# YamaneKoyo/mri-to-speech

Hardware: AMD Instinct MI355X
Metric: rtMRI frames/s end-to-end (256x256 frames -> 64-bin mel -> 11413 Hz wav) (higher is better)
Workload: dtype bf16x3; 1 GPU; e2e rtMRI->wav, 64 clips x 30 frames per GPU at 256x256 (configs[3] per-GPU share); clips_per_gpu=64, frames_per_clip=30, global_batch_clips=64, hw=256, parallelism=dp1, chunk=1920

## Files before the change

mri-to-speech_amd/csrc/acoustic_cnn.cpp:

```cpp
#include <algorithm>

#include "plan_util.hpp"
#include "prof.hpp"

namespace m2s {

Acoustic::Acoustic(const StateDict& sd, int n_mels, int hidden, int dtype, int device)
    : dtype_(dtype), device_(device), n_mels_(n_mels), hidden_(hidden), sw_(Switches::from_env()) {
  pack_acoustic(sd, n_mels, hidden, dtype, arena_, p_);
  arena_.upload(device);
  for (auto& b : p_.blocks) {
    b.c1.resolve(arena_);
    if (b.type != 0) b.c2.resolve(arena_);
    if (b.type == 2) {
      b.se1.resolve(arena_);
      b.se2.resolve(arena_);
    }
  }
  p_.lstm_ih.resolve(arena_);
  M2S_HIP(hipHostMalloc(reinterpret_cast<void**>(&err_host_), sizeof(unsigned), hipHostMallocMapped | hipHostMallocCoherent));
  *err_host_ = 0;
  M2S_HIP(hipHostGetDevicePointer(reinterpret_cast<void**>(&err_dev_), err_host_, 0));
  M2S_HIP(hipMalloc(&gsync_, lstm_sync_bytes(true)));
}
// ... 108 lines not shown
  const Block& b = p_.blocks[k];
  const BlockRoute& r = *p.r;
  const int nc = p.nc, oh = r.oh, ow = r.ow, nh = r.nh, nw = r.nw, qt = r.qt, ql = r.ql;
  T *const cur = p.cur, *const nxt = p.nxt;
  hipStream_t s = p.s;
  const int co = chan_stride(b.cout);
  const double px = (double)nc * nh * nw, flops = 2.0 * px * b.mid * (9.0 * b.cin + b.cout);
  if constexpr (kSplit<T>) {
    switch (r.er) {
      case ErRoute::ErSp:
        launch_er_sp(cur, nc, nh, nw, b.c1.cs_in, b.mid, co, arena_.ptr(b.er_sp_w), b.c1.b, b.c2.b, nxt, flops,
                     4.0 * px * (b.c1.cs_in + co), s, sw_.er_mrg);
        return;
      case ErRoute::Ers2Sp:
        launch_ers2_sp(cur, nc, oh, ow, nh, nw, qt, ql, b.c1.cs_in, b.mid, co, arena_.ptr(b.er_wexp), b.c1.b,
                       arena_.ptr(b.er_wpwl), b.c2.b, nxt, flops, 4.0 * ((double)nc * oh * ow * b.c1.cs_in + px * co), s);
        return;
      default:
        break;
    }
  } else if constexpr (std::is_same<T, bf16_t>::value) {
    const uint8_t* const x8 = r.x8_in ? p.cur8 : nullptr;
    uint8_t* const y8 = p.next8 = r.y8_out ? p.other8() : nullptr;
    switch (r.er) {
      case ErRoute::Er8:
        launch_er8_fused(cur, nc, nh, nw, arena_.at<uint8_t>(b.er8_wexp), arena_.at<float>(b.er8_sexp), b.c1.b,
                         arena_.at<uint8_t>(b.er8_wpwl), arena_.at<float>(b.er8_spwl), b.c2.b, nxt, flops,
                         2.0 * px * (2.0 * b.cin) + (3.0 * 8 * 2048 + 2 * 2048), s, x8, y8);
        return;
      case ErRoute::Er:
        launch_er_fused(cur, nc, nh, nw, arena_.at<bf16_t>(b.er_wexp), b.c1.b, arena_.at<bf16_t>(b.er_wpwl), b.c2.b, nxt,
                        flops, 2.0 * px * (2.0 * b.cin) + 2.0 * (9.0 * 32 * 128 + 128 * 32), s);
        return;
      case ErRoute::Er8w:
        launch_er8w_fused(cur, x8, nc, nh, nw, arena_.at<uint8_t>(b.er8w_w), arena_.at<float>(b.er8w_sexp), b.c1.b,
                          arena_.at<float>(b.er8w_spwl), b.c2.b, nxt, y8, flops,
                          px * (b.cin + 2.0 * b.cin + 2.0 * b.cout + (y8 ? b.cout : 0.0)) + (9.0 * b.cin + b.cout) * b.mid, s);
        return;
      case ErRoute::Er2:
        launch_er2_fused(cur, nc, nh, nw, arena_.at<bf16_t>(b.er_wexp), b.c1.b, b.c2.b, nxt, flops,
                         2.0 * px * (2.0 * b.c1.cs_in) + 2.0 * er2_stage_elems(), s);
        return;
      case ErRoute::Ers2:
        launch_ers2_fused(cur, nc, oh, ow, nh, nw, qt, ql, b.c1.cs_in, b.mid, co, arena_.at<bf16_t>(b.er_wexp), b.c1.b,
                          arena_.at<bf16_t>(b.er_wpwl), b.c2.b, nxt, flops,
                          2.0 * ((double)nc * oh * ow * b.c1.cs_in + px * co) + (y8 ? px * 32 : 0.0), s, y8);
        return;
      default:
        break;
    }
  }
  ConvArgs a = conv2d_args(p, b.c1, cur, p.b.M);
  a.act = ACT_SILU;
  ConvArgs q = pw_args(b.c2, p.b.M, nxt, nc * nh * nw, nh * nw);
  q.res = b.skip ? cur : nullptr;
  if (kSplit<T> && sw_.er_s2_fused && b.stride == 2 && conv_gemm_er_supported(a, q, sw_.conv)) {
    launch_conv_gemm_er(a, q, sw_.conv, s, flops,
                        4.0 * ((double)nc * oh * ow * b.cin + px * b.cout + (9.0 * b.cin + b.cout) * b.mid));
  } else {
    run_conv<T>(a, b.c1, sw_.conv, s);
    run_conv<T>(q, b.c2, sw_.conv, s);
  }
}

template <typename T>
void Acoustic::effnet_ir_front(EffPass<T>& p, size_t k) {
  const Block& b = p_.blocks[k];
  const BlockRoute& r = *p.r;
  const int nc = p.nc, oh = r.oh, ow = r.ow, nh = r.nh, nw = r.nw, qt = r.qt, ql = r.ql;
  T *const cur = p.cur, *const M = p.b.M, *const M2 = p.b.M2, *const se_mean = p.b.se_mean;
  float* const sums = p.b.sums;
  hipStream_t s = p.s;
  const int cs = chan_stride(b.mid);
  constexpr bool SPL = kSplit<T>;
  const bool f8 = r.f8;
  const float *const dw_w = arena_.at<float>(b.dw_w), *const dw_b = arena_.at<float>(b.dw_b);
  const void* wdw = SPL ? dw_w : arena_.ptr(b.dw_w2);
  const double Po = (double)nh * nw, es = SPL ? 4.0 : 2.0;
  auto ir_ws = [&](int ih, int iw, int stride, int OH, int OW, int pad_t, int pad_l) {
    const double Pi = (double)ih * iw;
    launch_ir_ws(cur, nc, ih, iw, b.c1.cs_in, b.c1.kp, cs, b.c1.w, b.c1.b, dw_w, dw_b, M2, se_mean,
                 2.0 * nc * b.mid * (Pi * b.c1.cin + Po * 9),
                 4.0 * nc * Pi * b.c1.cin + 4.0 * b.mid * (b.c1.cin + 11.0) + 4.0 * nc * b.mid, s, ws_report(), stride,
                 OH, OW, pad_t, pad_l, 4.0 * nc * Po * b.mid, r.mid_f32, sw_.irws_parts);
  };
  if (r.convert8) {
    p.cur8 = p.b.X8[0];
    launch_rows_e4m3(cur, (long)nc * oh * ow, b.c1.cs_in, p.cur8, b.f8x_kp, s);
  }
  const uint8_t* const x8 = r.x8_in ? p.cur8 : nullptr;
  const double Pi = (double)oh * ow;
  switch (r.front) {
    case IrFront::IrWs:
      ir_ws(nh, nw, 1, 0, 0, 0, 0);
      break;
    case IrFront::Pwdw:
      launch_ir_pwdw(cur, nc, b.c1.cs_in, b.c1.kp, b.c1.w, b.c1.b, wdw, dw_b, nh, nw, cs, M2, se_mean, SPL,
                     2.0 * nc * Po * b.mid * (b.c1.cin + 9), nc * Po * ((x8 ? 1.0 : es) * b.c1.cin + (f8 ? 1.0 : es) * b.mid),
                     s, f8, x8, x8 ? arena_.ptr(b.f8x_w) : nullptr, x8 ? arena_.at<float>(b.f8x_s) : nullptr, b.f8x_kp);
      break;
    case IrFront::IrWsS2:
      ir_ws(oh, ow, 2, nh, nw, qt, ql);
      break;
    case IrFront::PwdwS2:
      launch_ir_pwdw_s2(cur, nc, b.c1.cs_in, b.c1.kp, b.c1.w, b.c1.b, wdw, dw_b, oh, ow, nh, nw, qt, ql, cs, M2, se_mean,
                        SPL, 2.0 * nc * b.mid * (Pi * b.c1.cin + Po * 9),
                        nc * ((x8 ? 1.0 : es) * Pi * b.c1.cin + (f8 ? 1.0 : es) * Po * b.mid), s, f8, x8,
                        x8 ? arena_.ptr(b.f8x_w) : nullptr, x8 ? arena_.at<float>(b.f8x_s) : nullptr, b.f8x_kp);
      break;
    case IrFront::S2Band: {
      launch_ir_s2band(cur, nc, oh, ow, b.c1.cs_in, b.c1.kp, b.c1.w, b.c1.b, dw_w, dw_b, nh, nw, qt, ql, cs, M2, sums, SPL,
                       2.0 * nc * b.mid * (Pi * 1.125 * b.c1.cin + Po * 9),
                       nc * (es * Pi * b.c1.cs_in + (f8 ? 1.0 : es) * Po * cs), s, f8);
      ProfScope ps(tname<T>("se_mean_kernel"), 0.0, 4.0 * nc * cs * ir_s2band_bands(nh) + es * nc * cs, s);
      launch_se_mean<T>(sums, nc, ir_s2band_bands(nh), cs, 1.0f / (float)(nh * nw), se_mean, s);
      break;
    }
    case IrFront::Unfused: {
      ConvArgs e = pw_args(b.c1, cur, M, nc * oh * ow, oh * ow);
      e.act = ACT_SILU;
      run_conv<T>(e, b.c1, sw_.conv, s);
      {
        ProfScope ps(b.stride == 2 ? tname<T>("dwconv_kernel", ", 2") : tname<T>("dwconv_kernel", ", 1"), 2.0 * nc * nh * nw * b.mid * 9,
                     kStoreBytes<T> * (double)nc * (oh * ow + nh * nw) * b.mid, s);
        launch_dwconv<T>(M, nc, oh, ow, nh, nw, b.stride, qt, ql, b.mid, cs, dw_w, dw_b, M2, sums, s);
      }
      {
        ProfScope ps(tname<T>("se_mean_kernel"), 0.0, 4.0 * nc * cs * dw_pixel_blocks(nh, nw) + kStoreBytes<T> * (double)nc * cs, s);
        launch_se_mean<T>(sums, nc, dw_pixel_blocks(nh, nw), cs, 1.0f / (float)(nh * nw), se_mean, s);
      }
      break;
    }
  }
}

template <typename T>
void Acoustic::effnet_ir_se(EffPass<T>& p, size_t k) {
  const Block& b = p_.blocks[k];
  const int nc = p.nc, cs = chan_stride(b.mid);
  T *const se_mean = p.b.se_mean, *const se_hid = p.b.se_hid, *const scale = p.b.scale;
  hipStream_t s = p.s;
  switch (p.r->se) {
    case IrSe::Excite:
      launch_se_excite(se_mean, nc, b.mid, cs, b.se1.w, b.se1.kp, b.se1.b, b.rd, b.se2.w, b.se2.kp, b.se2.b, scale,
                       kSplit<T>, s);
      break;
    case IrSe::Convs: {
      ConvArgs r1 = pw_args(b.se1, se_mean, se_hid, nc, 1);
      r1.act = ACT_SILU;
      run_conv<T>(r1, b.se1, sw_.conv, s);
      ConvArgs r2 = pw_args(b.se2, se_hid, scale, nc, 1);
      r2.act = ACT_SIGMOID;
      run_conv<T>(r2, b.se2, sw_.conv, s);
      break;
    }
  }
}

template <typename T>
void Acoustic::effnet_ir_pwl(EffPass<T>& p, size_t k) {
  const Block& b = p_.blocks[k];
  const BlockRoute& r = *p.r;
  const int nc = p.nc, nh = r.nh, nw = r.nw, cs = chan_stride(b.mid), co = chan_stride(b.cout);
  T *const cur = p.cur, *const nxt = p.nxt, *const M2 = p.b.M2, *const scale = p.b.scale;
  hipStream_t s = p.s;
  uint8_t* const next8 = p.next8 = r.y8_out ? p.other8() : nullptr;
  const int ld8 = r.ld8;
// ... 133 lines not shown
```

mri-to-speech_amd/csrc/ir_ws.hip:

```cpp
#include <algorithm>
#include <cstdlib>
#include <type_traits>
#include <vector>

#include "kernels.hpp"
#include "lds_dma.hpp"
#include "prof.hpp"

namespace m2s {
namespace {

constexpr int WS_SL = 32;
constexpr int WS_BR = 8;
constexpr int WS_NP = 8;
constexpr int WS_NC = 8;
constexpr int WS_UMAX = 3;

__device__ __forceinline__ int hx_of(int r) { return ((r & 3) << 2) | swz_f((r >> 2) & 3); }

struct WsLayout {
  int XR, TROWS, x_bytes, tile_bytes, w_bytes, total;
};

__host__ __device__ inline int ws_cpp(int cs_in) { return (cs_in * 2 + 255) / 256 * 16; }
__host__ __device__ inline WsLayout ws_layout(int H, int W, int cs_in, int cs_mid, int S = 1) {
  WsLayout L;
  const int cpp = ws_cpp(cs_in), xp = 2 * cpp * 16;
  L.XR = 0;
  for (int r0 = 0; r0 < H; r0 += WS_BR) {
    const int a = r0 > 0 ? r0 - 1 : 0, b = r0 + WS_BR + 1 < H ? r0 + WS_BR + 1 : H;
    L.XR = b - a > L.XR ? b - a : L.XR;
  }
  const int tr = ((H < WS_BR ? H : WS_BR) + 2) * (W + 2);
  L.TROWS = S == 1 ? tr + (20 - tr % 16) % 16 : tr + (21 - tr % 16) % 16;
  L.x_bytes = L.XR * W * xp;
  L.tile_bytes = 2 * 8 * L.TROWS * 16;
  L.w_bytes = 2 * (cs_in / 32) * 4096;
  L.total = L.x_bytes + L.tile_bytes + L.w_bytes + (3 * 320 + 2 * 32) * 4 + cs_mid * 8 + 2 * (cs_mid / WS_SL) * 4 + 128;
  return L;
}

#ifndef IRWS_HAND_END
#define IRWS_HAND_END 2
#endif
#ifndef IRWS_PF_DEEP
#define IRWS_PF_DEEP 1
#endif
#ifndef IRWS_PAIR
#define IRWS_PAIR 1
#endif
#ifndef IRWS_TAPS_AHEAD
#define IRWS_TAPS_AHEAD 1
#endif
#ifndef IRWS_JOINT
#define IRWS_JOINT 1
#endif
#ifndef IRWS_PAR
#define IRWS_PAR 1
#endif
template <int W, int KS, int S>
__global__ void __launch_bounds__(64 * (WS_NP + WS_NC), 1)
    ir_ws_kernel(const bf16_t* __restrict__ x, int N, int H, int cs_mid, const bf16_t* __restrict__ wpw,
                 const float* __restrict__ bpw, const float* __restrict__ wdw, const float* __restrict__ bdw,
                 bf16_t* __restrict__ y, bf16_t* __restrict__ se_mean, unsigned long long* __restrict__ trace,
                 unsigned spin_max, unsigned* __restrict__ err, int pad_t, int pad_l, int fm32, int n_full, int parts) {
  constexpr int par = IRWS_PAR;
  static_assert(S == 1 || (S == 2 && W == 16), "stride 2: the 16-wide maps");
  constexpr int OWS = W / S;
  constexpr int OPB = (WS_BR / S) * OWS;
  constexpr bool HAND_END = IRWS_HAND_END == 2 ? W == 8 : IRWS_HAND_END, TAPS_AHEAD = IRWS_TAPS_AHEAD;
  constexpr bool JOINT = IRWS_JOINT && !HAND_END && (IRWS_JOINT == 2 || S == 2);
  constexpr int CS = KS * 32;
  constexpr int CPP = (CS * 2 + 255) / 256 * 16;
  constexpr int CPR = 2 * CPP;
  constexpr int XP = CPR * 16;
  constexpr int WT = W + 2;
  constexpr int WS_PXL = WS_BR * W / 64;
  extern __shared__ __attribute__((aligned(16))) char smem[];
  const WsLayout Lg = ws_layout(H, W, CS, cs_mid, S);
  const int NB = (H + WS_BR - 1) / WS_BR, NS = cs_mid / WS_SL, P = H * W;
  const int PO = S == 1 ? P : ((H + 1) / 2) * OWS;
  const int PLT = Lg.TROWS * 16;
  char* xs = smem;
  char* tiles = xs + Lg.x_bytes;
  char* wbuf = tiles + Lg.tile_bytes;
  float* wdl = reinterpret_cast<float*>(wbuf + Lg.w_bytes);
  float* bpl = wdl + 3 * 320;
  unsigned long long* sq = reinterpret_cast<unsigned long long*>(bpl + 2 * 32);
  unsigned* sq_n = reinterpret_cast<unsigned*>(sq + cs_mid);
  unsigned* sq_nan = sq_n + cs_mid / WS_SL;
  unsigned* ctr = reinterpret_cast<unsigned*>(smem + Lg.total - 128);
  unsigned* pdone = ctr + 0;
  unsigned* wrdy = ctr + 1;
  unsigned* xrdy = ctr + 2;
  unsigned* tfull = ctr + 3;
  unsigned* poison = ctr + 4;
  unsigned* tfree = ctr + 8;

  const int tid = threadIdx.x, lane = tid & 63;
  const int wave = __builtin_amdgcn_readfirstlane(tid >> 6);
  const int g = lane >> 4, r16 = lane & 15;
  const bool prod = wave < WS_NP;
  const int pw = wave & 1;
  unsigned* const pdone_p = par ? (pw ? ctr + 5 : ctr + 0) : pdone;
  unsigned* const wrdy_p = par ? (pw ? ctr + 6 : ctr + 1) : wrdy;
  const unsigned NPC = par ? WS_NP / 2 : WS_NP;
  const int n_units = n_full + (N - n_full) * parts;
  struct Unit {
    int img, lo, hi;
  };
  auto unit_of = [&](int u) {
    if (u < n_full) return Unit{u, 0, NS};
    const int q = u - n_full, pt = q % parts;
    return Unit{n_full + q / parts, pt * NS / parts, (pt + 1) * NS / parts};
  };
  int T = 0;
  for (int u = blockIdx.x; u < n_units; u += gridDim.x) {
    const Unit un = unit_of(u);
    T += NB * (un.hi - un.lo);
  }

  auto TR = [&](int i, int k) {
#ifdef IRWS_TRACE
    if (trace && blockIdx.x == 0 && i < 64) {
      const unsigned long long t = __builtin_amdgcn_s_memtime();
      if (lane == 0) trace[((i * 2 + (wave >= WS_NP)) * 16 + k) * 64 + (wave & 7)] = t;
    }
#else
    (void)i; (void)k; (void)trace;
#endif
  };
  struct Step {
    int img, band, sl, lo, hi, u;
  };
  auto first_step = [&](int u) {
    const Unit un = unit_of(u);
    return Step{un.img, 0, un.lo, un.lo, un.hi, u};
  };
  auto next_step = [&](Step d) {
    if (++d.sl == d.hi) {
      d.sl = d.lo;
      if (++d.band == NB) d = first_step(d.u + (int)gridDim.x);
    }
    return d;
  };

  if (tid < 32) ctr[tid] = 0u;
  for (int i = tid; i < cs_mid; i += 64 * (WS_NP + WS_NC)) sq[i] = 0ull;
// ... 320 lines not shown
    if (__builtin_amdgcn_readfirstlane(arrived) == (unsigned)(NB * WS_NC - 1) && lane < WS_SL) {
      const unsigned long long t = __hip_atomic_exchange(sq + c0 + sc, 0ull, __ATOMIC_RELAXED, __HIP_MEMORY_SCOPE_WORKGROUP);
      const float m = __fmaf_rn((float)(unsigned)t, 2.3283064365386963e-10f, (float)(int)(t >> 32)) / (float)PO;
      act_st<sp_t>(reinterpret_cast<sp_t*>(se_mean), d.img, cs_mid, c0 + sc, (*poison || sq_nan[d.sl]) ? __builtin_nanf("") : m);
      if (lane == 0) {
        sq_n[d.sl] = 0u;
        sq_nan[d.sl] = 0u;
      }
    }
  };

  __syncthreads();
  if (prod) {
    __builtin_amdgcn_s_setprio(2);
    Step cur = first_step(blockIdx.x);
    if (T > 0) issue_w(0, cur);
    if (T > 1) issue_w(1, next_step(cur));
    if (TAPS_AHEAD && T > 0 && tap_wave) issue_wd(0, cur);
    if (T > 0) {
      wait_vm_le((T > 1 ? npw : 0) + (TAPS_AHEAD && tap_wave ? 1 : 0));
      bump(wrdy_p);
      if (!HAND_END) wait_ge(wrdy_p, NPC);
    }
    static_assert(4 * KS <= 4 * WS_NP, "pieces per wave");
    int bands = 0;
    for (int i = 0; i < T; ++i) {
      const Step nxt = next_step(cur), nxt2 = next_step(nxt);
      TR(i, 0);
      if (cur.sl == cur.lo) {
        if (i > 0) {
          wait_ge(pdone_p, NPC * (unsigned)i);
          if (par) wait_ge(pw ? ctr + 0 : ctr + 5, NPC * (unsigned)i);
        }
        issue_x(cur.img, cur.band);
        wait_vm<0>();
        bump(xrdy);
        wait_ge(xrdy, (unsigned)(WS_NP * ++bands));
      }
      TR(i, 1);
      if (!TAPS_AHEAD && tap_wave) {
        if (i >= 3) wait_all(tfree, (unsigned)(i - 2));
        issue_wd(i, cur);
      }
      if (HAND_END) wait_ge(wrdy_p, NPC * (unsigned)(i + 1));
      TR(i, 2);
      produce(i, cur, nxt2);
      if (HAND_END) {
        wait_vm<0>();
        asm volatile("s_waitcnt lgkmcnt(0)" ::: "memory");
        if (lane == 0) {
          asm volatile("ds_add_u32 %0, %1" ::"v"((uint32_t)(uintptr_t)wrdy_p), "v"(1u) : "memory");
          asm volatile("ds_add_u32 %0, %1" ::"v"((uint32_t)(uintptr_t)tfull), "v"(1u) : "memory");
        }
        TR(i, 12);
        const bool nw = i + 2 < T, nt = TAPS_AHEAD && tap_wave && i + 1 < T;
        if (nw || nt) {
          wait_ge(pdone_p, NPC * (unsigned)(i + 1));
          if (nw) issue_w(i + 2, nxt2);
          if (nt) issue_wd(i + 1, nxt);
        }
      } else {
        if (tap_wave) {
          const bool nt = TAPS_AHEAD && i + 1 < T;
          if (nt) issue_wd(i + 1, nxt);
          wait_vm_le((i + 2 < T ? npw : 0) + (nt ? 1 : 0));
        }
        bump(tfull);
        TR(i, 12);
      }
      TR(i, 3);
      cur = nxt;
    }
  } else {
    Step cur = first_step(blockIdx.x);
    for (int i = 0; i < T; ++i) {
      wait_ge(tfull, (unsigned)(WS_NP * (i + 1)));
      consume(i, cur);
      TR(i, 7);
      cur = next_step(cur);
    }
  }
}

#ifdef IRWS_TRACE
static void dump_trace(unsigned long long* tr, hipStream_t s, const char* tag) {
  static int calls = 0;
  if (++calls > 40) return;
  std::vector<unsigned long long> h(64 * 2 * 16 * 64);
  M2S_HIP(hipStreamSynchronize(s));
  M2S_HIP(hipMemcpy(h.data(), tr, h.size() * 8, hipMemcpyDeviceToHost));
  auto at = [&](int i, int c, int k, int w = 0) { return (long long)h[((i * 2 + c) * 16 + k) * 64 + w]; };
  fprintf(stderr, "TRACE %s:", tag);
  for (int i = 2; i < 12; ++i)
    fprintf(stderr, " [P x %lld wr %lld mfma %lld tf %lld epi %lld hand %lld | C wait %lld px %lld bump %lld shf %lld at %lld]",
            at(i, 0, 1) - at(i, 0, 0), at(i, 0, 2) - at(i, 0, 1), at(i, 0, 6) - at(i, 0, 2), at(i, 0, 9) - at(i, 0, 6),
            at(i, 0, 12) - at(i, 0, 9), at(i, 0, 3) - at(i, 0, 12), at(i, 1, 4) - at(i - 1, 1, 7), at(i, 1, 5) - at(i, 1, 4),
            at(i, 1, 10) - at(i, 1, 5), at(i, 1, 11) - at(i, 1, 10), at(i, 1, 7) - at(i, 1, 11));
  fprintf(stderr, "\n");
  fprintf(stderr, "TRACEW %s:", tag);
  for (int i = 2; i < 4; ++i) {
    fprintf(stderr, " [s%d", i);
    for (int w = 0; w < 8; ++w) {
      fprintf(stderr, " w%d", w);
      for (int k : {0, 2, 6, 9, 12, 3}) fprintf(stderr, "%c%lld", k ? '/' : ' ', at(i, 0, k, w) - at(i, 0, 0));
    }
    fprintf(stderr, "]");
  }
  fprintf(stderr, "\n");
  fprintf(stderr, "TRACEC %s:", tag);
  for (int i = 4; i < 7; ++i) {
    fprintf(stderr, " [s%d P0 mfma_end %lld vm0 %lld pdone %lld after %lld tf %lld tfull %lld |", i, at(i, 0, 6) - at(i, 0, 0),
            at(i, 0, 13) - at(i, 0, 0), at(i, 0, 14) - at(i, 0, 0), at(i, 0, 8) - at(i, 0, 0), at(i, 0, 9) - at(i, 0, 0),
            at(i, 0, 12) - at(i, 0, 0));
    for (int j = i - 2; j <= i; ++j) {
      fprintf(stderr, " c%d:", j);
      for (int w = 0; w < 8; ++w)
        fprintf(stderr, " %lld/%lld/%lld", at(j, 1, 4, w) - at(i, 0, 0), at(j, 1, 10, w) - at(i, 0, 0), at(j, 1, 7, w) - at(i, 0, 0));
    }
    fprintf(stderr, "]");
  }
  fprintf(stderr, "\n");
  M2S_HIP(hipMemset(tr, 0, h.size() * 8));
}
#endif

}

bool ir_ws_s2_supported(int H, int W, int cs_in, int kp, int cs_mid, int OH, int OW, int pad_t, int pad_l) {
  return H == 16 && W == 16 && OH == 8 && OW == 8 && pad_t >= 0 && pad_t <= 1 && pad_l >= 0 && pad_l <= 1 &&
         ir_ws_supported(H, W, cs_in, kp, cs_mid) && ws_layout(H, W, cs_in, cs_mid, 2).total <= 160 * 1024;
}

bool ir_ws_supported(int H, int W, int cs_in, int kp, int cs_mid) {
  if (!((W == 8 && (kp == 128 || kp == 224)) || (W == 16 && kp == 128)) || H < 1 || H > 64 || cs_in != kp) return false;
  if (cs_mid % WS_SL != 0 || cs_mid < 3 * WS_SL) return false;
  const WsLayout L = ws_layout(H, W, cs_in, cs_mid);
  const int cpr = 2 * ws_cpp(cs_in);
  return L.total <= 160 * 1024 && (L.XR * W * cpr) % 64 == 0 && L.XR * W * cpr / 64 / WS_NP + 1 <= 60 &&
         2 * ((L.XR * W + 15) / 16) <= WS_NP * WS_UMAX;
}

void launch_ir_ws(const void* x, int N, int H, int W, int cs_in, int kp, int cs_mid, const void* wpw, const float* bpw,
                  const float* wdw, const float* bdw, void* y, void* se_mean, double flops, double bytes,
                  hipStream_t s, AsyncReport rep, int stride, int OH, int OW, int pad_t, int pad_l, double spill,
                  bool fm32, int forced_parts) {
  M2S_CHECK(stride == 1 ? ir_ws_supported(H, W, cs_in, kp, cs_mid)
                        : stride == 2 && ir_ws_s2_supported(H, W, cs_in, kp, cs_mid, OH, OW, pad_t, pad_l),
            "ir_ws: unsupported shape");
  M2S_CHECK(N > 0, "ir_ws: no images");
  M2S_CHECK((double)N * H * W * cs_mid * 4.0 < 4294967296.0, "ir_ws: output map too large for 32-bit offsets");
  const WsLayout L = ws_layout(H, W, cs_in, cs_mid, stride);
  const int n_cu = device_cus();
  const dim3 grid(std::min(N, n_cu));
  const int G = (int)grid.x, NSl = cs_mid / WS_SL;
  const int n_full = N / G * G, rem = N - n_full;
  int parts = rem > 0 ? std::max(1, (G + rem / 2) / rem) : 1;
  parts = std::max(1, std::min(parts, NSl / 3));
  if (forced_parts > 0) parts = std::min(forced_parts, std::max(1, NSl / 3));
#ifdef IRWS_TRACE
  static unsigned long long* tr = [] {
    unsigned long long* p = nullptr;
    if (getenv("M2S_IR_WS_TRACE")) M2S_HIP(hipMalloc(&p, 64 * 2 * 16 * 64 * 8));
    return p;
  }();
#define M2S_IRWS_DUMP(tag) \
  if (tr) dump_trace(tr, s, tag);
#else
  unsigned long long* tr = nullptr;
#define M2S_IRWS_DUMP(tag)
#endif
  const bf16_t* xb = static_cast<const bf16_t*>(x);
  const bf16_t* wb = static_cast<const bf16_t*>(wpw);
  bf16_t* yb = static_cast<bf16_t*>(y);
  bf16_t* mb = static_cast<bf16_t*>(se_mean);
#define M2S_IRWS(W_, KS_, S_, NAME_)                                                                    \
  if (W == W_ && kp == KS_ * 32 && stride == S_) {                                                      \
    allow_lds(reinterpret_cast<const void*>(&ir_ws_kernel<W_, KS_, S_>));                             \
    ProfScope ps(NAME_, flops, bytes, s, spill);                                                        \
    hipLaunchKernelGGL((ir_ws_kernel<W_, KS_, S_>), grid, dim3(64 * (WS_NP + WS_NC)), L.total, s, xb, N, H, cs_mid, wb, \
                       bpw, wdw, bdw, yb, mb, tr, rep.spin_max, rep.err, pad_t, pad_l, fm32 ? 1 : 0, n_full, parts); \
    M2S_IRWS_DUMP(NAME_)                                                                                \
    M2S_HIP(hipGetLastError());                                                                         \
    return;                                                                                             \
  }
  M2S_IRWS(8, 4, 1, "ir_ws_kernel<8, 4, 1>") M2S_IRWS(8, 7, 1, "ir_ws_kernel<8, 7, 1>")
  M2S_IRWS(16, 4, 1, "ir_ws_kernel<16, 4, 1>") M2S_IRWS(16, 4, 2, "ir_ws_kernel<16, 4, 2>")
#undef M2S_IRWS
#undef M2S_IRWS_DUMP
  M2S_CHECK(false, "ir_ws: no variant for this shape");
}

}
```

mri-to-speech_amd/csrc/kernels.hpp:

```cpp
#pragma once

#include "lstm_route.hpp"
#include "m2s_common.hpp"

namespace m2s {

enum AsyncCode : unsigned { M2S_ASYNC_LSTM = 1u, M2S_ASYNC_WS = 2u };
struct AsyncReport {
  unsigned spin_max = 1u << 20;
  unsigned* err = nullptr;
};
__device__ __forceinline__ void report_async(unsigned* err, unsigned code, int lane) {
  if (err && lane == 0) __hip_atomic_store(err, code, __ATOMIC_RELAXED, __HIP_MEMORY_SCOPE_SYSTEM);
}

template <typename T>
void launch_stem(const float* frames, int N, int H, int W, int OH, int OW, int pad_t, int pad_l,
                 const float* w9, const float* bias, int cout, int cs_out, T* y, hipStream_t s);

int dw_pixel_blocks(int OH, int OW);
template <typename T>
void launch_dwconv(const T* x, int N, int IH, int IW, int OH, int OW, int stride, int pad_t, int pad_l,
                   int C, int cs, const float* w9, const float* bias, T* y, float* sums, hipStream_t s);

template <typename T>
void launch_se_mean(const float* psum, int N, int npb, int cs, float inv_count, T* mean, hipStream_t s);

bool ir_fused_supported(int OH, int OW, int cs_in, int cs_mid, bool split);
void launch_ir_pwdw(const void* x, int N, int cs_in, int kp, const void* wpw, const float* bpw, const void* wdw,
                    const float* bdw, int OH, int OW, int cs_mid, void* y, void* se_mean, bool split, double flops,
                    double bytes, hipStream_t s, bool f8_out = false, const void* x8 = nullptr,
                    const void* w8 = nullptr, const float* wsc = nullptr, int kp8 = 0);
void launch_rows_e4m3(const void* x, long rows, int cs, void* y8, int ld8, hipStream_t s);

bool se_gemm_f8_supported(int P, int cs_in, int cs_out);
void launch_se_gemm_f8(const void* x8, int M, int P, int cs_in, const void* w8, int kp, int n_pad, const float* wscale,
                       const float* bias, const void* gate, const void* res, void* y, int cs_out, hipStream_t s,
                       double flops, double bytes, void* y8 = nullptr, int ld8 = 0);

bool se_gemm_sp_supported(int P, int cs_in, int cs_out);
void launch_se_gemm_sp(const void* x, int M, int P, int cs_in, const void* w, int n_pad, const float* bias,
                       const void* gate, const void* res, void* y, int cs_out, hipStream_t s, double flops, double bytes,
                       int waves);

bool se_ws_supported(int P, int cs_in, int cs_out);
void launch_se_ws(const void* x, int M, int P, int cs_in, const void* w, int n_pad, const float* bias, const void* gate,
                  const void* res, void* y, int cs_out, hipStream_t s, double flops, double bytes, AsyncReport rep,
                  bool x_f32, bool rev, bool half, int cfg);

bool se_ws_f8_supported(int P, int cs_in, int cs_out);
void launch_se_ws_f8(const void* x8, int M, int P, int cs_in, const void* w8, int kp, int n_pad, const float* wscale,
                     const float* bias, const void* gate, const void* res, void* y, int cs_out, hipStream_t s, double flops,
                     double bytes, void* y8 = nullptr, int ld8 = 0, AsyncReport rep = {}, bool half = false);

bool ir_ws_supported(int H, int W, int cs_in, int kp, int cs_mid);
bool ir_ws_s2_supported(int H, int W, int cs_in, int kp, int cs_mid, int OH, int OW, int pad_t, int pad_l);
void launch_ir_ws(const void* x, int N, int H, int W, int cs_in, int kp, int cs_mid, const void* wpw, const float* bpw,
                  const float* wdw, const float* bdw, void* y, void* se_mean, double flops, double bytes,
                  hipStream_t s, AsyncReport rep = {}, int stride = 1, int OH = 0, int OW = 0, int pad_t = 0,
                  int pad_l = 0, double spill = 0.0, bool fm32 = false, int parts = 0);
int ir_s2band_bands(int OH);
bool ir_s2band_supported(int IH, int IW, int OH, int OW, int cs_in, int kp, int cs_mid);
void launch_ir_s2band(const void* x, int N, int IH, int IW, int cs_in, int kp, const void* wpw, const float* bpw,
                      const float* wdw, const float* bdw, int OH, int OW, int pad_t, int pad_l, int cs_mid, void* y,
                      float* psum, bool split, double flops, double bytes, hipStream_t s, bool f8_out = false);
bool ir_fused_s2_supported(int IH, int IW, int cs_in, int cs_mid, bool split);
void launch_ir_pwdw_s2(const void* x, int N, int cs_in, int kp, const void* wpw, const float* bpw, const void* wdw,
                       const float* bdw, int IH, int IW, int OH, int OW, int pad_t, int pad_l, int cs_mid, void* y,
                       void* se_mean, bool split, double flops, double bytes, hipStream_t s, bool f8_out = false,
                       const void* x8 = nullptr, const void* w8 = nullptr, const float* wsc = nullptr, int kp8 = 0);

bool conv1d_halo_sp_supported(int C, int cs, int k, int dil);
size_t conv1d_halo_frag_elems(int C, int k);
void launch_conv1d_halo_sp(const struct ConvArgs* a, int n, hipStream_t s, double flops, double bytes);
struct HaloPair {
  const void* x;
  const void* w1;
  const void* w2;
  const float* b1;
  const float* b2;
  void* y;
  int k, dil;
  int accum;
  int act;
};
bool conv1d_halo_pair_supported(int C, int cs, int k, int dil);
bool conv1d_halo_pair_fills(int C, int B, int L);
void launch_conv1d_halo_pair(const HaloPair* p, int n, int C, int B, int L, bool chain, float div, hipStream_t s,
                             double flops, double bytes);
bool rb1_fused_supported(int C, int cs, int k, const int* dil, int np, int kp, bool split);
int rb1_frag_taps(int C, int k, bool split);
void launch_rb1_fused(const bf16_t* x, bf16_t* s, int B, int L, int C, int k, int np, const int* dil,
                      const bf16_t* const* w1, const float* const* b1, const bf16_t* const* w2,
                      const float* const* b2, int kp, int accum, float div, bool split, double flops, double bytes,
                      hipStream_t st);

void launch_stem_b0(const float* frames, int N, int H, int W, int OH, int OW, int pad_t, int pad_l, const float* w9,
                    const float* b9, const void* w0, const float* b0, int kp0, const void* w1, const float* b1,
                    int kp1, void* y, bool split, double flops, double bytes, hipStream_t s, int parts);

bool se_excite_supported(int rd, int kp2, int cs_mid);
void launch_se_excite(const void* mean, int N, int mid, int cs_mid, const void* w1, int kp1, const float* b1,
                      int rd, const void* w2, int kp2, const float* b2, void* gate, bool split, hipStream_t s);

bool er_fused_supported(int H, int W, int cin, int mid, int cout, int kp_exp, int kp_pwl);
void launch_er_fused(const bf16_t* x, int N, int H, int W, const bf16_t* wexp, const float* bexp, const bf16_t* wpwl,
                     const float* bpwl, bf16_t* y, double flops, double bytes, hipStream_t s);

bool er8_fused_supported(int H, int W, int cin, int mid, int cout);
void launch_er8_fused(const bf16_t* x, int N, int H, int W, const uint8_t* wexp, const float* sexp, const float* bexp,
                      const uint8_t* wpwl, const float* spwl, const float* bpwl, bf16_t* y, double flops, double bytes,
                      hipStream_t s, const uint8_t* x8 = nullptr, uint8_t* y8 = nullptr);

bool er2_fused_supported(int H, int W, int cs_in, int mid, int cout, int kp_exp, int kp_pwl);
int er2_stage_elems();
bool er8w_fused_supported(int H, int W, int cs_in, int mid, int cout);
size_t er8w_stream_bytes();
void launch_er8w_fused(const bf16_t* x, const uint8_t* x8, int N, int H, int W, const uint8_t* wst, const float* sexp,
                       const float* bexp, const float* spwl, const float* bpwl, bf16_t* y, uint8_t* y8, double flops,
                       double bytes, hipStream_t s);
void launch_er2_fused(const bf16_t* x, int N, int H, int W, const bf16_t* wst, const float* bexp, const float* bpwl,
                      bf16_t* y, double flops, double bytes, hipStream_t s);

bool er_sp_supported(int H, int W, int cs_in, int mid, int cs_out);
int er_sp_nt_stages(int cs_in, int mid, int cs_out, int* nt);
void launch_er_sp(const void* x, int N, int H, int W, int cs_in, int mid, int cs_out, const void* wst, const float* bexp,
                  const float* bpwl, void* y, double flops, double bytes, hipStream_t s, bool merged = true);

bool ers2_fused_supported(int OH, int OW, int cs_in, int mid, int cs_out, int kp_exp, int kp_pwl);
int ers2_exp_elems(int cs_in, int mid);
bool ers2_sp_supported(int OH, int OW, int cs_in, int mid, int cs_out);
void launch_ers2_sp(const void* x, int N, int H, int W, int OH, int OW, int pad_t, int pad_l, int cs_in, int mid,
                    int cs_out, const void* wexp, const float* bexp, const void* wpwl, const float* bpwl, void* y,
                    double flops, double bytes, hipStream_t s);
void launch_ers2_fused(const bf16_t* x, int N, int H, int W, int OH, int OW, int pad_t, int pad_l, int cs_in, int mid,
                       int cs_out, const bf16_t* wexp, const float* bexp, const bf16_t* wpwl, const float* bpwl,
                       bf16_t* y, double flops, double bytes, hipStream_t s, uint8_t* y8 = nullptr);

void launch_preprocess(const uint8_t* frames, int N, int H, int W, int channels, float* out, hipStream_t s);

void launch_frames(const uint8_t* frames, int N, int h, int w, int channels, int out_h, int out_w, int interp, int norm,
                   float* out, hipStream_t s);
void launch_frames_masked(const uint8_t* frames, int N, int h, int w, int channels, const float* masks, int n_masks,
// ... 86 lines not shown
```

mri-to-speech_amd/csrc/switches.hpp:

```cpp
#pragma once

#include <algorithm>
#include <cstdlib>
#include <cstring>

namespace m2s {

struct ConvTune {
  int ksplit = 0;
  int ksplit_max = 8;
  int ksplit_minst = 4;
  bool bn64 = false;
  int stages = 0;
};

struct Switches {
  bool ir_fused = true;
  bool ir_ws = true;
  bool ir_ws_s2 = true;
  bool irws_f32 = true;
  bool stem_fused = true;
  bool f8_er = true;
  bool se_y8 = true;
  bool f8_er2 = true;
  bool er8_x8 = true;
  bool f8_expand = true;
  bool f8_s2 = true;
  bool se_fused = true;
  bool er_fused = true;
  bool se_sp = false;
  bool se_ws = true;
  bool er_mrg = true;
  bool ir_s2band = true;
  bool er_s2_fused = true;
  bool sews_rev = true;

  int irws_min = 512;
  int sews_min_cus = 1;
  int irws_parts = 0;
  int stem_parts = 0;
  bool sews_half = false;
  int se_ws_cfg = 0;
  int se_sp_waves = 8;

  bool lstm_persistent = true;
  bool lstm_mid = true;
  bool lstm_x3 = true;
  bool lstm_x3g = true;
  int lstm_small_b = 4;
  int lstm_mid_ch = 0;

  bool mrf_fused = true;
  bool mrf_halo = true;
  bool mrf_pair = true;
  bool mrf_chain = true;
  bool mrf_pair128 = false;
  bool f8_mrf64 = false;
  bool f8_mrf32 = false;
  bool mrf_batch = true;

  ConvTune conv;

  template <class Seen>
  static Switches from_env(Seen seen);
  static Switches from_env() {
    return from_env([](const char*) {});
  }
};

inline void env_flag(const char* name, bool& v) {
  if (const char* e = std::getenv(name)) v = std::strcmp(e, "0") != 0;
}
inline bool env_int(const char* name, int& v) {
  const char* e = std::getenv(name);
  if (e) v = std::atoi(e);
  return e != nullptr;
}

template <class Seen>
Switches Switches::from_env(Seen seen) {
  Switches w;
  auto flag = [&](const char* name, bool& v) {
    seen(name);
    env_flag(name, v);
  };
  auto num = [&](const char* name, int& v) {
    seen(name);
    return env_int(name, v);
  };
  auto val = [&](const char* name) {
    int v = 0;
    num(name, v);
    return v;
  };
  flag("M2S_IR_FUSED", w.ir_fused);
  flag("M2S_IR_WS", w.ir_ws);
  flag("M2S_IR_WS_S2", w.ir_ws_s2);
  flag("M2S_IRWS_F32", w.irws_f32);
  flag("M2S_STEM_FUSED", w.stem_fused);
  flag("M2S_F8_EXPAND", w.f8_expand);
  flag("M2S_F8_S2", w.f8_s2);
  flag("M2S_F8_ER", w.f8_er);
  flag("M2S_ER8_X8", w.er8_x8);
  flag("M2S_F8_ER2", w.f8_er2);
  flag("M2S_SE_Y8", w.se_y8);
  flag("M2S_SE_FUSED", w.se_fused);
  flag("M2S_ER_FUSED", w.er_fused);
  flag("M2S_SE_WS", w.se_ws);
  flag("M2S_SE_SP", w.se_sp);
  flag("M2S_ER_MRG", w.er_mrg);
  flag("M2S_IR_S2BAND", w.ir_s2band);
  flag("M2S_ER_S2_FUSED", w.er_s2_fused);
  flag("M2S_SEWS_REV", w.sews_rev);
  num("M2S_IRWS_MIN", w.irws_min);
  num("M2S_SEWS_MIN", w.sews_min_cus);
  num("M2S_IRWS_PARTS", w.irws_parts);
  if (int p = 0; num("M2S_STEM_PARTS", p)) w.stem_parts = std::max(1, p);
  w.sews_half = val("M2S_SEWS_HALF") == 1;
  num("M2S_SE_WS_CFG", w.se_ws_cfg);
  w.se_sp_waves = val("M2S_SE_SP_WAVES") == 4 ? 4 : 8;
  flag("M2S_LSTM_PERSISTENT", w.lstm_persistent);
  flag("M2S_LSTM_MID", w.lstm_mid);
  flag("M2S_LSTM_X3", w.lstm_x3);
  flag("M2S_LSTM_X3G", w.lstm_x3g);
  w.lstm_small_b = val("M2S_LSTM_SMALL_B") == 8 ? 8 : 4;
  if (const int ch = val("M2S_LSTM_MID_CH"); ch == 4 || ch == 8 || ch == 16) w.lstm_mid_ch = ch;
  flag("M2S_MRF_FUSED", w.mrf_fused);
  flag("M2S_MRF_BATCH", w.mrf_batch);
  flag("M2S_MRF_HALO", w.mrf_halo);
  flag("M2S_F8_MRF64", w.f8_mrf64);
  flag("M2S_F8_MRF32", w.f8_mrf32);
  flag("M2S_MRF_PAIR", w.mrf_pair);
  flag("M2S_MRF_CHAIN", w.mrf_chain);
  flag("M2S_MRF_PAIR128", w.mrf_pair128);
  num("M2S_KSPLIT", w.conv.ksplit);
  if (num("M2S_KSPLIT_MAX", w.conv.ksplit_max)) w.conv.ksplit_max = std::max(1, w.conv.ksplit_max);
  if (num("M2S_KSPLIT_MINST", w.conv.ksplit_minst)) w.conv.ksplit_minst = std::max(1, w.conv.ksplit_minst);
  w.conv.bn64 = val("M2S_CG_BN64") == 1;
  num("M2S_CG_STAGES", w.conv.stages);
  return w;
}

}
```

Before: 51210 rtMRI frames/s.

## Replace producer/consumer handoff with per-wave fused kernel for 16-wide IR blocks

For stride-1 16x16 inverted-residual blocks with H<=16, the previous warp-specialized kernel (producer waves handing tiles to consumer waves through LDS with spin flags) is swapped for a new kernel. In it each of 8 waves owns 16-channel groups end to end: bf16x3 MFMA pointwise expansion, then a depthwise 3x3 computed in registers using DPP lane shifts, then the SE mean. Taps and weights for the next group are prefetched while the current group's epilogue runs, and the input image is DMA'd into LDS once per unit. The intent is to remove handoff synchronisation and LDS round-trips. The cost is heavier register use per wave and a new code path that the old form can still be selected over via M2S_IR_WS=handoff.

```diff
diff --git a/mri-to-speech_amd/csrc/acoustic_cnn.cpp b/mri-to-speech_amd/csrc/acoustic_cnn.cpp
--- a/mri-to-speech_amd/csrc/acoustic_cnn.cpp
+++ b/mri-to-speech_amd/csrc/acoustic_cnn.cpp
@@ -214,7 +214,7 @@
     launch_ir_ws(cur, nc, ih, iw, b.c1.cs_in, b.c1.kp, cs, b.c1.w, b.c1.b, dw_w, dw_b, M2, se_mean,
                  2.0 * nc * b.mid * (Pi * b.c1.cin + Po * 9),
                  4.0 * nc * Pi * b.c1.cin + 4.0 * b.mid * (b.c1.cin + 11.0) + 4.0 * nc * b.mid, s, ws_report(), stride,
-                 OH, OW, pad_t, pad_l, 4.0 * nc * Po * b.mid, r.mid_f32, sw_.irws_parts);
+                 OH, OW, pad_t, pad_l, 4.0 * nc * Po * b.mid, r.mid_f32, sw_.irws_parts, sw_.irws_handoff);
   };
   if (r.convert8) {
     p.cur8 = p.b.X8[0];
diff --git a/mri-to-speech_amd/csrc/ir_ws.hip b/mri-to-speech_amd/csrc/ir_ws.hip
--- a/mri-to-speech_amd/csrc/ir_ws.hip
+++ b/mri-to-speech_amd/csrc/ir_ws.hip
@@ -59,11 +59,13 @@
 #define IRWS_PAR 1
 #endif
 template <int W, int KS, int S>
-__global__ void __launch_bounds__(64 * (WS_NP + WS_NC), 1)
-    ir_ws_kernel(const bf16_t* __restrict__ x, int N, int H, int cs_mid, const bf16_t* __restrict__ wpw,
-                 const float* __restrict__ bpw, const float* __restrict__ wdw, const float* __restrict__ bdw,
-                 bf16_t* __restrict__ y, bf16_t* __restrict__ se_mean, unsigned long long* __restrict__ trace,
-                 unsigned spin_max, unsigned* __restrict__ err, int pad_t, int pad_l, int fm32, int n_full, int parts) {
+__device__ __forceinline__ void ir_ws_handoff(const bf16_t* __restrict__ x, int N, int H, int cs_mid,
+                                              const bf16_t* __restrict__ wpw, const float* __restrict__ bpw,
+                                              const float* __restrict__ wdw, const float* __restrict__ bdw,
+                                              bf16_t* __restrict__ y, bf16_t* __restrict__ se_mean,
+                                              unsigned long long* __restrict__ trace, unsigned spin_max,
+                                              unsigned* __restrict__ err, int pad_t, int pad_l, int fm32, int n_full,
+                                              int parts) {
   constexpr int par = IRWS_PAR;
   static_assert(S == 1 || (S == 2 && W == 16), "stride 2: the 16-wide maps");
   constexpr int OWS = W / S;
@@ -550,6 +552,28 @@
   }
 }
 
+#include "ir_ws_wave.hpp"
+
+constexpr bool ws_wave_shape(int W, int S) { return W == 16 && S == 1; }
+template <int W, int KS, int S>
+__global__ void __launch_bounds__(ws_wave_shape(W, S) ? 64 * WV_NW : 64 * (WS_NP + WS_NC), 1)
+    ir_ws_kernel(const bf16_t* __restrict__ x, int N, int H, int cs_mid, const bf16_t* __restrict__ wpw,
+                 const float* __restrict__ bpw, const float* __restrict__ wdw, const float* __restrict__ bdw,
+                 bf16_t* __restrict__ y, bf16_t* __restrict__ se_mean, unsigned long long* __restrict__ trace,
+                 unsigned spin_max, unsigned* __restrict__ err, int pad_t, int pad_l, int fm32, int n_full, int parts) {
+  if constexpr (ws_wave_shape(W, S)) ir_ws_wave16<KS>(x, N, H, cs_mid, wpw, bpw, wdw, bdw, y, se_mean, fm32, n_full, parts);
+  else ir_ws_handoff<W, KS, S>(x, N, H, cs_mid, wpw, bpw, wdw, bdw, y, se_mean, trace, spin_max, err, pad_t, pad_l, fm32, n_full, parts);
+}
+template <int W, int KS, int S, int HANDOFF>
+__global__ void __launch_bounds__(64 * (WS_NP + WS_NC), 1)
+    ir_ws_kernel(const bf16_t* __restrict__ x, int N, int H, int cs_mid, const bf16_t* __restrict__ wpw,
+                 const float* __restrict__ bpw, const float* __restrict__ wdw, const float* __restrict__ bdw,
+                 bf16_t* __restrict__ y, bf16_t* __restrict__ se_mean, unsigned long long* __restrict__ trace,
+                 unsigned spin_max, unsigned* __restrict__ err, int pad_t, int pad_l, int fm32, int n_full, int parts) {
+  static_assert(HANDOFF == 1, "the handed-off form");
+  ir_ws_handoff<W, KS, S>(x, N, H, cs_mid, wpw, bpw, wdw, bdw, y, se_mean, trace, spin_max, err, pad_t, pad_l, fm32, n_full, parts);
+}
+
 #ifdef IRWS_TRACE
 static void dump_trace(unsigned long long* tr, hipStream_t s, const char* tag) {
   static int calls = 0;
@@ -611,7 +635,7 @@
 void launch_ir_ws(const void* x, int N, int H, int W, int cs_in, int kp, int cs_mid, const void* wpw, const float* bpw,
                   const float* wdw, const float* bdw, void* y, void* se_mean, double flops, double bytes,
                   hipStream_t s, AsyncReport rep, int stride, int OH, int OW, int pad_t, int pad_l, double spill,
-                  bool fm32, int forced_parts) {
+                  bool fm32, int forced_parts, bool handoff) {
   M2S_CHECK(stride == 1 ? ir_ws_supported(H, W, cs_in, kp, cs_mid)
                         : stride == 2 && ir_ws_s2_supported(H, W, cs_in, kp, cs_mid, OH, OW, pad_t, pad_l),
             "ir_ws: unsupported shape");
@@ -641,18 +665,26 @@
   const bf16_t* wb = static_cast<const bf16_t*>(wpw);
   bf16_t* yb = static_cast<bf16_t*>(y);
   bf16_t* mb = static_cast<bf16_t*>(se_mean);
-#define M2S_IRWS(W_, KS_, S_, NAME_)                                                                    \
-  if (W == W_ && kp == KS_ * 32 && stride == S_) {                                                      \
-    allow_lds(reinterpret_cast<const void*>(&ir_ws_kernel<W_, KS_, S_>));                             \
+  const bool wave_form = ws_wave_shape(W, stride) && H <= 16 && !handoff;
+#define M2S_IRWS_GO(KERNEL_, THREADS_, LDS_, NAME_)                                                     \
+  {                                                                                                     \
+    allow_lds(reinterpret_cast<const void*>(&KERNEL_));                                                 \
     ProfScope ps(NAME_, flops, bytes, s, spill);                                                        \
-    hipLaunchKernelGGL((ir_ws_kernel<W_, KS_, S_>), grid, dim3(64 * (WS_NP + WS_NC)), L.total, s, xb, N, H, cs_mid, wb, \
-                       bpw, wdw, bdw, yb, mb, tr, rep.spin_max, rep.err, pad_t, pad_l, fm32 ? 1 : 0, n_full, parts); \
+    hipLaunchKernelGGL((KERNEL_), grid, dim3(THREADS_), LDS_, s, xb, N, H, cs_mid, wb, bpw, wdw, bdw, yb, mb, tr, \
+                       rep.spin_max, rep.err, pad_t, pad_l, fm32 ? 1 : 0, n_full, parts);               \
     M2S_IRWS_DUMP(NAME_)                                                                                \
     M2S_HIP(hipGetLastError());                                                                         \
     return;                                                                                             \
   }
+  if (ws_wave_shape(W, stride) && kp == 128) {
+    if (wave_form) M2S_IRWS_GO((ir_ws_kernel<16, 4, 1>), 64 * WV_NW, WV_NW * 1024 + H * W * 2 * ws_cpp(cs_in) * 16, "ir_ws_kernel<16, 4, 1>")
+    M2S_IRWS_GO((ir_ws_kernel<16, 4, 1, 1>), 64 * (WS_NP + WS_NC), L.total, "ir_ws_kernel<16, 4, 1, 1>")
+  }
+#define M2S_IRWS(W_, KS_, S_, NAME_)                                                                    \
+  if (W == W_ && kp == KS_ * 32 && stride == S_) M2S_IRWS_GO((ir_ws_kernel<W_, KS_, S_>), 64 * (WS_NP + WS_NC), L.total, NAME_)
   M2S_IRWS(8, 4, 1, "ir_ws_kernel<8, 4, 1>") M2S_IRWS(8, 7, 1, "ir_ws_kernel<8, 7, 1>")
-  M2S_IRWS(16, 4, 1, "ir_ws_kernel<16, 4, 1>") M2S_IRWS(16, 4, 2, "ir_ws_kernel<16, 4, 2>")
+  M2S_IRWS(16, 4, 2, "ir_ws_kernel<16, 4, 2>")
+#undef M2S_IRWS_GO
 #undef M2S_IRWS
 #undef M2S_IRWS_DUMP
   M2S_CHECK(false, "ir_ws: no variant for this shape");
diff --git a/mri-to-speech_amd/csrc/ir_ws_wave.hpp b/mri-to-speech_amd/csrc/ir_ws_wave.hpp
--- /dev/null
+++ b/mri-to-speech_amd/csrc/ir_ws_wave.hpp
@@ -0,0 +1,237 @@
+#pragma once
+
+
+#ifndef IRWS_WAVE_ABL
+#define IRWS_WAVE_ABL 0
+#endif
+constexpr int WV_NW = 8;
+constexpr int WV_GC = 16;
+constexpr int WV_PF = 5;
+
+__device__ __forceinline__ float dpp_left(float v) {
+  return __builtin_bit_cast(float, __builtin_amdgcn_update_dpp(0, __builtin_bit_cast(int, v), 0x111, 0xF, 0xF, true));
+}
+__device__ __forceinline__ float dpp_right(float v) {
+  return __builtin_bit_cast(float, __builtin_amdgcn_update_dpp(0, __builtin_bit_cast(int, v), 0x101, 0xF, 0xF, true));
+}
+template <int ROR>
+__device__ __forceinline__ float dpp_ror_add(float v) {
+  return v + __builtin_bit_cast(float, __builtin_amdgcn_update_dpp(0, __builtin_bit_cast(int, v), 0x120 + ROR, 0xF, 0xF, false));
+}
+
+template <int KS, bool FULL, bool F32>
+__device__ __forceinline__ void ir_ws_wave16(const bf16_t* __restrict__ x, int N, int H, int cs_mid,
+                                             const bf16_t* __restrict__ wpw, const float* __restrict__ bpw,
+                                             const float* __restrict__ wdw, const float* __restrict__ bdw,
+                                             bf16_t* __restrict__ y, bf16_t* __restrict__ se_mean, int n_full, int parts) {
+  constexpr int W = 16, HMAX = 16;
+  constexpr int CS = KS * 32;
+  constexpr int CPP = (CS * 2 + 255) / 256 * 16;
+  constexpr int CPR = 2 * CPP;
+  constexpr int XP = CPR * 16;
+  extern __shared__ __attribute__((aligned(16))) char smem[];
+  char* xs = smem + WV_NW * 1024;
+  const int tid = threadIdx.x, lane = tid & 63;
+  const int wave = __builtin_amdgcn_readfirstlane(tid >> 6);
+  const int g = lane >> 4, r16 = lane & 15;
+  const int NG = cs_mid / WV_GC, P = H * W;
+  const int n_units = n_full + (N - n_full) * parts;
+  const char* zpage = zero_page();
+  const int hxl = hx_of(r16);
+
+  struct AFrag {
+    bf16x8 h[KS], l[KS];
+  };
+  auto lane_now = [&]() {
+    int ln = lane;
+    asm volatile("" : "+v"(ln));
+    return ln;
+  };
+  auto load_a = [&](int cg) {
+    AFrag a;
+    const int ln = lane_now();
+    const bf16_t* wr = wpw + ((size_t)(cg * WV_GC + (ln & 15)) * CS * 2 + (ln >> 4) * 8);
+#pragma unroll
+    for (int ks = 0; ks < KS; ++ks) {
+      a.h[ks] = *reinterpret_cast<const bf16x8*>(wr + ks * 32);
+      a.l[ks] = *reinterpret_cast<const bf16x8*>(wr + CS + ks * 32);
+    }
+    return a;
+  };
+
+  struct Taps {
+    float4 w[9], bp, bd;
+  };
+  char* const tslot = smem + wave * 1024;
+  auto issue_taps = [&](int cg) {
+    const int ln = lane_now(), t = ln >> 2, c = cg * WV_GC + 4 * (ln & 3);
+    const void* src = t < 9 ? static_cast<const void*>(wdw + (t * cs_mid + c))
+                            : t == 9 ? static_cast<const void*>(bpw + c) : t == 10 ? static_cast<const void*>(bdw + c) : zpage;
+    dma16_asm(src, lds_lo32_u(tslot));
+  };
+  auto read_taps = [&]() {
+    Taps t;
+#pragma unroll
+    for (int k = 0; k < 9; ++k) t.w[k] = *reinterpret_cast<const float4*>(tslot + k * 64 + g * 16);
+    t.bp = *reinterpret_cast<const float4*>(tslot + 9 * 64 + g * 16);
+    t.bd = *reinterpret_cast<const float4*>(tslot + 10 * 64 + g * 16);
+    return t;
+  };
+
+  for (int u = blockIdx.x; u < n_units; u += gridDim.x) {
+    int img = u, glo = 0, ghi = NG;
+    if (u >= n_full) {
+      const int q = u - n_full, pt = q % parts;
+      img = n_full + q / parts;
+      glo = pt * NG / parts;
+      ghi = (pt + 1) * NG / parts;
+    }
+    int cg = glo + wave;
+    AFrag a;
+    if (cg < ghi) {
+      issue_taps(cg);
+      a = load_a(cg);
+    }
+    __syncthreads();
+    if (!(IRWS_WAVE_ABL & 4) || u == (int)blockIdx.x) {
+      const int ninstr = P * CPR / 64;
+      const bf16_t* xi = x + (size_t)img * P * CS * 2;
+      for (int j = wave; j < ninstr; j += WV_NW) {
+        const int id = j * 64 + lane, r = id / CPR, p = id - r * CPR;
+        const int L = (p & ~15) | ((p & 15) ^ hx_of(r));
+        const int plane = L / CPP, k8 = L - plane * CPP;
+        const void* src = k8 * 8 < CS ? static_cast<const void*>(xi + (size_t)r * CS * 2 + plane * CS + k8 * 8) : zpage;
+        dma16_asm(src, lds_lo32_u(xs + j * 1024));
+      }
+    }
+    __builtin_amdgcn_s_waitcnt(0x0F70);
+    asm volatile("" ::: "memory");
+    __syncthreads();
+
+    auto unit = [&]() {
+      const int c4 = cg * WV_GC + 4 * g;
+      f32x4 acc[HMAX];
+      {
+        constexpr int NI = HMAX * KS;
+        bf16x8 bh[WV_PF], bl[WV_PF];
+        auto load_b = [&](int i) {
+          const int T = i / KS, ks = i % KS;
+          const char* xr = xs + (T * 16 + r16) * XP;
+          const int Lh = ks * 4 + g, Ll = CPP + ks * 4 + g;
+          const int ph = ((Lh & ~15) | ((Lh & 15) ^ hxl)) << 4, pl = ((Ll & ~15) | ((Ll & 15) ^ hxl)) << 4;
+          bh[i % WV_PF] = *reinterpret_cast<const bf16x8*>(xr + ph);
+          bl[i % WV_PF] = *reinterpret_cast<const bf16x8*>(xr + pl);
+        };
+#pragma unroll
+        for (int i = 0; i < WV_PF - 1; ++i)
+          if (FULL || i / KS < H) load_b(i);
+#pragma unroll
+        for (int i = 0; i < NI; ++i) {
+          const int T = i / KS, ks = i % KS, ip = i + WV_PF - 1;
+          if (FULL || T < H) {
+            if (ip < NI && (FULL || ip / KS < H)) load_b(ip);
+            __builtin_amdgcn_sched_barrier(0);
+            f32x4 c = ks == 0 ? f32x4{0.f, 0.f, 0.f, 0.f} : acc[T];
+            c = __builtin_amdgcn_mfma_f32_16x16x32_bf16(a.l[ks], bh[i % WV_PF], c, 0, 0, 0);
+            c = __builtin_amdgcn_mfma_f32_16x16x32_bf16(a.h[ks], bl[i % WV_PF], c, 0, 0, 0);
+            c = __builtin_amdgcn_mfma_f32_16x16x32_bf16(a.h[ks], bh[i % WV_PF], c, 0, 0, 0);
+            acc[T] = c;
+          }
+        }
+      }
+      __builtin_amdgcn_sched_barrier(0);
+      asm volatile("" ::: "memory");
+      const Taps tp = read_taps();
+      asm volatile("s_waitcnt lgkmcnt(0)" ::: "memory");
+      const int cgn = cg + WV_NW < ghi ? cg + WV_NW : cg;
+      issue_taps(cgn);
+      const AFrag an = load_a(cgn);
+      __builtin_amdgcn_sched_barrier(0);
+
+      const uint32_t ps = 4u * (uint32_t)cs_mid;
+      const int lny = lane_now();
+      const uint32_t ylane = (uint32_t)(lny & 15) * ps + (F32 ? 4u * (uint32_t)(cg * WV_GC + 4 * (lny >> 4))
+                                                              : 128u * (uint32_t)(cg >> 1) + 8u * (uint32_t)((cg & 1) * 4 + (lny >> 4)));
+      char* const yimg = reinterpret_cast<char*>(y) + (uint32_t)(img * P) * ps;
+      float sum[4] = {0.f, 0.f, 0.f, 0.f};
+      const float bbv[4] = {tp.bp.x, tp.bp.y, tp.bp.z, tp.bp.w}, bdv[4] = {tp.bd.x, tp.bd.y, tp.bd.z, tp.bd.w};
+      float w[9][4];
+#pragma unroll
+      for (int t = 0; t < 9; ++t) {
+        w[t][0] = tp.w[t].x; w[t][1] = tp.w[t].y; w[t][2] = tp.w[t].z; w[t][3] = tp.w[t].w;
+      }
+      float prv[4] = {0.f, 0.f, 0.f, 0.f}, cur[4] = {bdv[0], bdv[1], bdv[2], bdv[3]}, nxt[4] = {0.f, 0.f, 0.f, 0.f};
+#pragma unroll
+      for (int s = 0; s <= HMAX; ++s) {
+        if ((IRWS_WAVE_ABL & 2) && s < HMAX && (FULL || s < H)) {
+#pragma unroll
+          for (int j = 0; j < 4; ++j) nxt[j] = silu(acc[s][j] + bbv[j]) + w[4][j];
+        } else if (s < HMAX && (FULL || s < H)) {
+#pragma unroll
+          for (int j = 0; j < 4; ++j) {
+            const float uc = silu(acc[s][j] + bbv[j]);
+            const float ul = dpp_left(uc), ur = dpp_right(uc);
+            nxt[j] = bdv[j];
+            nxt[j] += w[0][j] * ul;
+            nxt[j] += w[1][j] * uc;
+            nxt[j] += w[2][j] * ur;
+            cur[j] += w[3][j] * ul;
+            cur[j] += w[4][j] * uc;
+            cur[j] += w[5][j] * ur;
+            if (s > 0) {
+              prv[j] += w[6][j] * ul;
+              prv[j] += w[7][j] * uc;
+              prv[j] += w[8][j] * ur;
+            }
+          }
+        }
+        if (s >= 1 && (FULL || s - 1 < H)) {
+          float o[4];
+#pragma unroll
+          for (int j = 0; j < 4; ++j) {
+            o[j] = silu(prv[j]);
+            sum[j] += o[j];
+          }
+          char* dst = yimg + ((uint32_t)(s - 1) * 16u * ps + ylane);
+          if (IRWS_WAVE_ABL & 1) {
+          } else if (F32) {
+            *reinterpret_cast<float4*>(dst) = make_float4(o[0], o[1], o[2], o[3]);
+          } else {
+            uint2 hi, lo;
+            split4(o, hi, lo);
+            *reinterpret_cast<uint2*>(dst) = hi;
+            *reinterpret_cast<uint2*>(dst + 64) = lo;
+          }
+        }
+#pragma unroll
+        for (int j = 0; j < 4; ++j) {
+          prv[j] = cur[j];
+          cur[j] = nxt[j];
+        }
+        __builtin_amdgcn_sched_barrier(0);
+      }
+
+#pragma unroll
+      for (int j = 0; j < 4; ++j) sum[j] = dpp_ror_add<1>(dpp_ror_add<2>(dpp_ror_add<4>(dpp_ror_add<8>(sum[j]))));
+      if (r16 < 4) {
+        const float v = r16 == 0 ? sum[0] : r16 == 1 ? sum[1] : r16 == 2 ? sum[2] : sum[3];
+        act_st<sp_t>(reinterpret_cast<sp_t*>(se_mean), img, cs_mid, c4 + r16, v / (float)P);
+      }
+      a = an;
+    };
+    for (; cg < ghi; cg += WV_NW) unit();
+  }
+}
+
+template <int KS>
+__device__ __forceinline__ void ir_ws_wave16(const bf16_t* __restrict__ x, int N, int H, int cs_mid,
+                                             const bf16_t* __restrict__ wpw, const float* __restrict__ bpw,
+                                             const float* __restrict__ wdw, const float* __restrict__ bdw,
+                                             bf16_t* __restrict__ y, bf16_t* __restrict__ se_mean, int fm32, int n_full,
+                                             int parts) {
+  const bool full = H == 16;
+  if (full && fm32) ir_ws_wave16<KS, true, true>(x, N, H, cs_mid, wpw, bpw, wdw, bdw, y, se_mean, n_full, parts);
+  else if (full) ir_ws_wave16<KS, true, false>(x, N, H, cs_mid, wpw, bpw, wdw, bdw, y, se_mean, n_full, parts);
+  else if (fm32) ir_ws_wave16<KS, false, true>(x, N, H, cs_mid, wpw, bpw, wdw, bdw, y, se_mean, n_full, parts);
+  else ir_ws_wave16<KS, false, false>(x, N, H, cs_mid, wpw, bpw, wdw, bdw, y, se_mean, n_full, parts);
+}
diff --git a/mri-to-speech_amd/csrc/kernels.hpp b/mri-to-speech_amd/csrc/kernels.hpp
--- a/mri-to-speech_amd/csrc/kernels.hpp
+++ b/mri-to-speech_amd/csrc/kernels.hpp
@@ -58,7 +58,7 @@
 void launch_ir_ws(const void* x, int N, int H, int W, int cs_in, int kp, int cs_mid, const void* wpw, const float* bpw,
                   const float* wdw, const float* bdw, void* y, void* se_mean, double flops, double bytes,
                   hipStream_t s, AsyncReport rep = {}, int stride = 1, int OH = 0, int OW = 0, int pad_t = 0,
-                  int pad_l = 0, double spill = 0.0, bool fm32 = false, int parts = 0);
+                  int pad_l = 0, double spill = 0.0, bool fm32 = false, int parts = 0, bool handoff = false);
 int ir_s2band_bands(int OH);
 bool ir_s2band_supported(int IH, int IW, int OH, int OW, int cs_in, int kp, int cs_mid);
 void launch_ir_s2band(const void* x, int N, int IH, int IW, int cs_in, int kp, const void* wpw, const float* bpw,
diff --git a/mri-to-speech_amd/csrc/switches.hpp b/mri-to-speech_amd/csrc/switches.hpp
--- a/mri-to-speech_amd/csrc/switches.hpp
+++ b/mri-to-speech_amd/csrc/switches.hpp
@@ -17,6 +17,7 @@
 struct Switches {
   bool ir_fused = true;
   bool ir_ws = true;
+  bool irws_handoff = false;
   bool ir_ws_s2 = true;
   bool irws_f32 = true;
   bool stem_fused = true;
@@ -95,6 +96,7 @@
   };
   flag("M2S_IR_FUSED", w.ir_fused);
   flag("M2S_IR_WS", w.ir_ws);
+  if (const char* e = std::getenv("M2S_IR_WS")) w.irws_handoff = std::strcmp(e, "handoff") == 0;
   flag("M2S_IR_WS_S2", w.ir_ws_s2);
   flag("M2S_IRWS_F32", w.irws_f32);
   flag("M2S_STEM_FUSED", w.stem_fused);
```

Result: faster. 53330 rtMRI frames/s (median of 6 runs) (+4.1%).
